# jianhao2016/AllSet

Measured on AMD Instinct MI355X. Metric: edges*d aggregated / sec (V->E->V layer fwd+bwd), higher is better.
Workload: dtype f32

## Files before the change

allset_amd/_lib.py:

```python
from __future__ import annotations

import ctypes
import os
from ctypes import c_char_p, c_float, c_int, c_int64, c_size_t, c_uint64, c_void_p, POINTER

import torch

LIB_PATH = os.path.join(os.path.dirname(os.path.abspath(__file__)), "liballset_hip.so")
ABI_VERSION = 15
CORE_ABI_VERSION = 1

SUM, MEAN, MAX, MIN = 0, 1, 2, 3
F32, BF16 = 0, 1
REDUCE_AS_TREE = 0x100
PACK_PITCH_DW, PACK_CAP = 64, 60
ARITH_AUTO, ARITH_BF16X6, ARITH_FP16X3 = 0, 1, 2
ACT_NONE, ACT_RELU, ACT_ELU = 0, 1, 2
REDUCE_CODES = {"add": SUM, "sum": SUM, "mean": MEAN, "max": MAX, "min": MIN}

_P = c_void_p
SIGNATURES = {
    "allset_version": [],
    "allset_core_version": [],
    "allset_csr_build_workspace_bytes": [c_int64, c_int64, POINTER(c_size_t)],
# ... 250 lines not shown
    "allset_spgemm_bool_fill": [_P, _P, _P, _P, c_int64, c_int64, c_int64, _P, c_int64, _P, _P, c_size_t, _P],
    "allset_loo_supported": [c_int64],
    "allset_loo_long_threshold": [],
    "allset_loo_rows": [_P, _P, _P, c_int64, _P, _P, _P, c_int64, _P, c_int64, c_int64, c_int64, c_int64, c_int64, _P],
    "allset_loo_softmax_supported": [c_int64, c_int64],
    "allset_loo_softmax_fwd": [_P, _P, _P, _P, c_int64, c_float, _P, c_int64, _P, _P, c_int64, c_int64, c_int64, c_int64, c_int64,
                               c_int64, _P],
    "allset_loo_softmax_bwd": [_P, _P, _P, _P, c_int64, c_float, _P, c_int64, _P, _P, c_int64, _P, _P, c_int64, _P, _P, _P, c_int64,
                               c_int64, c_int64, c_int64, c_int64, c_int64, _P],
    "allset_scan_rows_supported": [c_int64],
    "allset_scan_rows": [_P, _P, _P, c_int64, _P, _P, c_int64, _P, c_int64, c_int, c_int64, c_int64, c_int64, c_int64, _P],
    "allset_scan_collect": [_P, _P, _P, c_int64, _P, _P, c_int64, _P, _P, c_int, c_float, c_uint64, _P, _P, c_int64, c_int64, c_int64,
                            c_int64, c_int64, _P],
    "allset_pack_rows_f32": [_P, c_int64, _P, c_int64, c_int64, _P],
    "allset_segreduce_packed_fwd": [c_int, _P, _P, _P, _P, _P, c_int64, _P, c_int64, c_int64, c_int64, c_int64, _P],
}
EXPORTED_SYMBOLS = sorted(list(SIGNATURES) + ["allset_last_error"])


class AllSetHipError(RuntimeError):
    pass


_lib = None


def load() -> ctypes.CDLL:
    global _lib
    if _lib is not None:
        return _lib
# ... 71 lines not shown
```

allset_amd/csrc/fused_fwd2.hip:

```cpp
#include <stdlib.h>

#include "common.h"
#include "mfma.h"

namespace allset {

constexpr int kF2Block = 768;
constexpr int kF2Rows = 32;
constexpr int kF2VWaves = 8;
constexpr int kF2Sets = 4;

#ifdef ALLSET_ABL5_NOBAR
#define ALLSET_TICK() ALLSET_TICK_NO_BARRIER()
#else
#define ALLSET_TICK() ALLSET_TICK_BARRIER()
#endif

template <bool HAS_LN, bool DROP_IN, bool DROP_OUT, bool D8, bool F16, int XM = 0, bool AUX = false>
__global__ __launch_bounds__(kF2Block) void fused_linear_fwd_roles_kernel(
    const float* __restrict__ x, int64_t ldx, const float* __restrict__ gamma, const float* __restrict__ beta, float eps,
    int relu_in, float p_in, uint64_t seed_in, const float* __restrict__ W, const float* __restrict__ bias, int relu_out,
    float p_out, uint64_t seed_out, float* __restrict__ y, int64_t ldy, float* __restrict__ stats, int64_t n,
    const uint64_t* __restrict__ seed_base, uint32_t* __restrict__ mask_out, int64_t xcb, int64_t ycb, float ln_inv,
    const float* __restrict__ colb = nullptr, float* __restrict__ uo = nullptr, int64_t lduo = 0,
    const float* __restrict__ res = nullptr, int64_t ldres = 0, int relu_post = 0,
    const float* __restrict__ aux_w = nullptr, const float* __restrict__ aux_b = nullptr, float* __restrict__ aux_out = nullptr) {
  static_assert(!AUX || (XM == 0 && !DROP_IN && !HAS_LN), "auxiliary columns: the plain prologue only (behind a LayerNorm the fp16x3 form folds 2^Su into gamma / beta)");
  static_assert(XM == 0 || F16, "the tail modes are built on the fp16x3 arithmetic only");
  static_assert(XM != 1 || (HAS_LN && !DROP_IN && !DROP_OUT), "mode 1: LayerNorm prologue, no dropout");
  static_assert(XM != 2 || (!HAS_LN && !DROP_IN), "mode 2: plain operand, LayerNorm in the epilogue");
  constexpr bool ROWSC = F16 && !HAS_LN;
  constexpr bool AFF = HAS_LN || XM == 2;
  constexpr int KD = 128, ND = 128;
  constexpr int R = kF2Rows;
  constexpr int PLANE = R * 256;
  constexpr int IMG = 3 * PLANE;
  constexpr int SPY = 132;
  __shared__ __attribute__((aligned(16))) uint8_t sX[2 * IMG];
  __shared__ __attribute__((aligned(16))) float sY[2 * R * SPY];
  __shared__ __attribute__((aligned(16))) float sG[KD];
  __shared__ __attribute__((aligned(16))) float sB[KD];
  __shared__ __attribute__((aligned(16))) float sBias[ND];
  seed_in = resolve_seed(seed_base, seed_in);
// ... 240 lines not shown
          if (relu_post) { o.x = fmaxf(o.x, 0.f); o.y = fmaxf(o.y, 0.f); o.z = fmaxf(o.z, 0.f); o.w = fmaxf(o.w, 0.f); }
          if constexpr (DROP_OUT) {
            const float4 kp = keep4(seed_out, stage, hb, thr_out, keep_out);
            o.x *= kp.x; o.y *= kp.y; o.z *= kp.z; o.w *= kp.w;
          }
          if (live) *reinterpret_cast<float4*>(yb + hb * dhy + yo) = o;
        }
      }
#pragma unroll
      for (int hb = 0; hb < 2; ++hb) {
        float4 v = vv[hb];
        if constexpr (DROP_OUT && XM != 2) {
          const float4 kp = keep4(seed_out, stage, hb, thr_out, keep_out);
          v.x *= kp.x; v.y *= kp.y; v.z *= kp.z; v.w *= kp.w;
        }
#ifdef ALLSET_ABL5_NOSTORE
        if (live && v.x == 123.456f)
#else
        if (live && XM != 2)
#endif
          *reinterpret_cast<float4*>(yb + hb * dhy + yo) = v;
        if (mask_out != nullptr) {
          const uint64_t b0 = __ballot(v.x > 0.f), b1 = __ballot(v.y > 0.f), b2 = __ballot(v.z > 0.f), b3 = __ballot(v.w > 0.f);
          const int sh = 8 * (lane0 & 7);
          const uint32_t word = static_cast<uint32_t>((b0 >> sh) & 0xffu) | (static_cast<uint32_t>((b1 >> sh) & 0xffu) << 8) |
                                (static_cast<uint32_t>((b2 >> sh) & 0xffu) << 16) | (static_cast<uint32_t>((b3 >> sh) & 0xffu) << 24);
          if (lane0 < 8 && 16 * (wave >> 2) < nrows)
            mask_out[((stage * (R / 16) + (wave >> 2)) * (ND / 64) + hb) * 32 + (wave & 3) * 8 + lane0] = word;
        }
      }
      if constexpr (XM == 2) {
        __builtin_amdgcn_sched_barrier(0);
        request_res(k + 1);
        __builtin_amdgcn_sched_barrier(0);
      }
    };

    static_assert(kF2Sets == 4, "the trip below is written for four register sets");
#pragma unroll
    for (int q = 0; q < kF2Sets; ++q) request_x(q, xrS[q]);
    request_res(0);
    S0(0, xrS[0]);
    ALLSET_TICK();
// ... 199 lines not shown
    case 3: ALLSET_F2_K(false, true, true); break;
    case 4: ALLSET_F2_K(true, false, false); break;
    case 5: ALLSET_F2_K(true, false, true); break;
    case 6: ALLSET_F2_K(true, true, false); break;
    default: ALLSET_F2_K(true, true, true); break;
  }
#undef ALLSET_F2_K
#undef ALLSET_F2_KD
#undef ALLSET_F2_KE
  return 0;
}

static inline unsigned f2_grid(int64_t n) {
  const int64_t blocks = (n + kF2Rows - 1) / kF2Rows;
  return static_cast<unsigned>(blocks > 256 ? 256 : (blocks < 1 ? 1 : blocks));
}

extern "C" int allset_fused_linear_tail_supported(int64_t K, int64_t N) {
#ifdef ALLSET_NO_F16X3
  (void)K; (void)N;
  return 0;
#else
  return (K == 128 && N == 128) ? 1 : 0;
#endif
}

extern "C" int allset_fused_linear_fwd_ln_side(const float* x, int64_t ldx, const float* colb, const float* gamma, const float* beta,
                                               float eps, const float* W, const float* bias, int relu_out, float* y, int64_t ldy,
                                               float* uo, int64_t lduo, float* stats, int64_t n, int64_t K, int64_t N, void* stream) {
  clear_error();
// ... 57 lines not shown
```

allset_amd/dense.py:

```python
from __future__ import annotations

import contextlib
import os
from ctypes import byref, c_int64
from typing import Optional, Tuple

import torch
from torch.autograd.function import once_differentiable

from . import _lib
from ._lib import check, ptr, require_device, stream_of, on_device
from .ops import _ld, _rowmajor, _timed

Tensor = torch.Tensor


class _SeedSource:
    base: Optional[Tensor] = None
    salt: int = 0


_SEED_SCRATCH = torch.empty((), dtype=torch.int64)


# ... 1027 lines not shown
                                               mask is not None)):
            need = ctx.needs_input_grad
            defer = ctx.params if (_Deferred.active and (gamma is None or (need[1] and need[2])) and (not has_bias or need[4])) else None
            gx, dg, db, gw, gb = fused_linear_bwd_all(gy, mask, p_out, weight, x, stats, gamma, beta, relu_in, p_in, seed_in,
                                                      base, want_bias=need_b, defer_to=defer)
            return gx, dg, db, gw, gb, None, None, None, None, None, None, None
        if ctx.needs_input_grad[3] or need_b:
            gw, gb = wgrad_fused(gy, y, p_out, x, stats, gamma, beta, relu_in, p_in, seed_in, want_bias=need_b,
                                 seed_base=base, mask=mask)
        if ctx.needs_input_grad[0] or (gamma is not None and (ctx.needs_input_grad[1] or ctx.needs_input_grad[2])):
            gx, dg, db = fused_linear_bwd(gy, y, p_out, weight, x, stats, gamma, relu_in, p_in, seed_in, base, mask,
                                          want_gx=ctx.needs_input_grad[0])
        return gx, dg, db, gw, gb, None, None, None, None, None, None, None


class _WideNormLinear(torch.autograd.Function):

    @staticmethod
    def forward(ctx, x, gamma, beta, weight, bias, eps, relu_in, p_in, relu_out, p_out, stats_in=None, emit=None):
        seed_in = _draw_seed() if p_in > 0.0 else 0
        seed_out = _draw_seed() if p_out > 0.0 else 0
        base = _seed_base() if (p_in > 0.0 or p_out > 0.0) else None
        stats = (stats_in if stats_in is not None else row_stats(x, relu_in, eps)) if gamma is not None else None
        stats_y = torch.empty((x.shape[0], 2), dtype=torch.float32, device=x.device) if emit is not None else None
        keep_y = relu_out or p_out > 0.0
        words = activation_mask_words(x.shape[0], weight.shape[0]) if (keep_y and x.shape[0] > 0) else 0
        mask = torch.empty(words, dtype=torch.int32, device=x.device) if words > 0 else None
        y = gemm_x6(x, gemm_x6_planes(weight, False, f16=wide_f16(gamma is not None)), weight.shape[0], bias, relu_in=relu_in, stats=stats, gamma=gamma,
                    beta=beta, p_in=p_in, seed_in=seed_in, relu_out=relu_out, p_out=p_out, seed_out=seed_out, seed_base=base,
                    mask_out=mask, stats_out=stats_y, stats_eps=emit[0] if emit is not None else 1e-5,
# ... 1320 lines not shown
```

allset_amd/dist.py:

```python
from __future__ import annotations

import os
from typing import Callable, Optional, Tuple

import torch
import torch.distributed as dist
import torch.nn.functional as F

Tensor = torch.Tensor



def vertex_block(n_v: int, world: int, rank: int) -> Tuple[int, int, int]:
    per = (n_v + world - 1) // world
    return rank * per, (rank + 1) * per, per * world


def partition_hyperedges(sizes: Tensor, world: int, method: str = "contiguous") -> Tensor:
    sizes = sizes.to(torch.int64)
    n_e = sizes.numel()
    if method == "contiguous":
        csum = torch.cumsum(sizes, 0)
        total = int(csum[-1]) if n_e else 0
        mid = csum - sizes // 2
# ... 434 lines not shown
        T = inc.by_src
        return ops.pma_bwd_src(T.rowptr, T.col, alpha, V, gout, stats, slope,
                               variant=_variant(T, "pma_bwd_src", V.shape[0], V, alpha.shape[1]), row_order=T.row_order,
                               sizes=_sizes(T, V, alpha.shape[1]))


def _bn_scope(valid_rows: int, group):
    from . import dense
    return dense.sync_bn_rows(valid_rows, group)


def _valid_rows(lo: int, hi: int, n: int) -> int:
    return max(0, min(int(hi), int(n)) - int(lo))


def sharded_deepsets_layer(v2e_conv, e2v_conv, x_owned: Tensor, hg: ShardedHypergraph, aggr: str = "add",
                           dropout: float = 0.0, training: bool = False, group=None,
                           aggregate: Callable = _hip_deepsets, norm: Optional[Tensor] = None,
                           dropout_out: Optional[float] = None) -> Tensor:
    if aggr not in ("add", "sum", "mean", "max", "min"):
        raise ValueError(f"aggr {aggr!r}")
    vv = _valid_rows(hg.v_lo, hg.v_hi, hg.n_v)
    norm = hg.norm if norm is None else norm
    p_out = dropout if dropout_out is None else dropout_out
    use_halo = hg.halo is not None and hg.halo_v2e is not None
    agg_v2e, agg_e2v = _forward_aggregate(aggregate, v2e_conv), _forward_aggregate(aggregate, e2v_conv)
    with _bn_scope(vv, group):
        h = v2e_conv._mlp_act(v2e_conv.f_enc, x_owned, v2e_conv.dropout)
    if use_halo:
        e = agg_v2e(halo_gather(h, hg.halo), hg.halo_v2e, norm, aggr)
    else:
        h_full = all_gather_rows(h, group)
        e = agg_v2e(h_full, hg.v2e, norm, aggr)
    with _bn_scope(e.shape[0], group):
        e = v2e_conv._mlp_act(v2e_conv.f_dec, e, dropout)
        g = e2v_conv._mlp_act(e2v_conv.f_enc, e, e2v_conv.dropout)
    if aggr in ("max", "min") and use_halo:
        v = _HaloExtremeMerge.apply(agg_e2v(g, hg.halo_e2v, norm, aggr), hg, aggr == "min")
    elif aggr in ("max", "min"):
        partial = agg_e2v(g, hg.e2v, norm, aggr)
        v = _ShardedExtremeMerge.apply(partial, hg.local_vertex_has_incidence(), hg, group, aggr == "min")
    elif use_halo:
        v = halo_scatter_add(agg_e2v(g, hg.halo_e2v, norm, "add"), hg.halo)
    else:
        partial = agg_e2v(g, hg.e2v, norm, "add")
        v = reduce_scatter_rows(partial, group)
    if aggr == "mean":
        v = v / hg.owned_vertex_degree(group).clamp(min=1).view(-1, 1)
    with _bn_scope(vv, group):
        return e2v_conv._mlp_act(e2v_conv.f_dec, v, p_out)

# ... 752 lines not shown
```

allset_amd/functional.py:

```python
from __future__ import annotations

from typing import Optional, Tuple

import torch
from torch.autograd.function import once_differentiable

from . import _lib, ops
from ._lib import MAX, MEAN, MIN, REDUCE_CODES, SUM
from .incidence import Incidence, LeaveOneOutIncidence

Tensor = torch.Tensor


def _variant(csr, kind: str, n_rows: int, x: Tensor, heads: int = 1) -> int:
    es = x.element_size()
    wide = 16 // es
    d = x.shape[1]
    ok = (d % wide == 0 and d <= 64 * wide and x.stride(0) % wide == 0 and x.data_ptr() % 16 == 0
          and (d // max(heads, 1)) % wide == 0)
    if not ok:
        return 1
    if d * es <= 128 and csr.max_deg <= 512:
        return 2
    return csr.variant(kind, n_rows)
# ... 54 lines not shown
    return hit


_PACKED_GATHER = True


def set_packed_gather(on: bool) -> None:
    global _PACKED_GATHER
    _PACKED_GATHER = bool(on)


def packed_gather() -> bool:
    return _PACKED_GATHER


def _takes_packed(x: Tensor, w_dst: Optional[Tensor], inc: Incidence, reduce: int) -> bool:
    if not (_PACKED_GATHER and x.dtype == torch.float32 and x.dim() == 2 and x.shape[1] == 128 and x.is_contiguous()
            and x.data_ptr() % 16 == 0 and reduce in (SUM, MEAN) and w_dst is None and x.shape[0] > 0 and inc.n_dst > 0):
        return False
    csr = inc.by_dst
    return _variant(csr, "segreduce", inc.n_dst, x) == 1 and not (0 < _split(csr, x) < inc.n_dst)


class _SegReduce(torch.autograd.Function):
    @staticmethod
    def forward(ctx, x: Tensor, w_dst: Optional[Tensor], w_src: Optional[Tensor], inc: Incidence, reduce: int, packed_rows: bool = False):
        csr = inc.by_dst
        ext = reduce in (MAX, MIN)
        if packed_rows and _takes_packed(x, w_dst, inc, reduce):
            out = ops.segreduce_packed(reduce, csr.rowptr, csr.col, ops.pack_rows(x), x, inc.n_dst, row_order=csr.row_order)
            arg = None
        else:
            out, arg = ops.segreduce(reduce, csr.rowptr, csr.col, w_dst, x, inc.n_dst, want_arg=ext,
                                     variant=1 if ext else _variant(csr, "segreduce", inc.n_dst, x), row_order=csr.row_order,
                                     split=_split(csr, x))
        need_gw = w_dst is not None and ctx.needs_input_grad[1]
        ctx.inc, ctx.reduce, ctx.n_s, ctx.need_gw = inc, reduce, x.shape[0], need_gw
        ctx.save_for_backward(x if need_gw else None, w_dst, w_src, arg)
        return out

    @staticmethod
    @once_differentiable
    def backward(ctx, gout: Tensor):
        x, w_dst, w_src, arg = ctx.saved_tensors
# ... 8 lines not shown
        if ctx.needs_input_grad[0]:
            if w_dst is not None and w_src is None:
                w_src = w_dst[inc.pos_dst_of_src().long()]
            if reduce in (SUM, MEAN):
                if reduce == MEAN:
                    inv = inc.inv_count_by_src()
                    w_src = inv if w_src is None else w_src * inv
                gx, _ = ops.segreduce(SUM, T.rowptr, T.col, w_src, gout, ctx.n_s,
                                      variant=_variant(T, "segreduce", ctx.n_s, gout), row_order=T.row_order,
                                      split=_split(T, gout) if ctx.n_s == T.n_rows else -1)
            else:
                gx = ops.segmax_bwd(T.rowptr, T.col, inc.pos_dst_of_src(), w_src, arg, gout, ctx.n_s)
        if ctx.need_gw:
            csr = inc.by_dst
            gw = ops.sddmm_rowdot(reduce, csr.rowptr, csr.col, x, gout, arg)
        return gx, gw, None, None, None, None


def deepsets_aggregate(x: Tensor, inc: Incidence, norm: Optional[Tensor] = None, aggr: str = "add",
                       packed_rows: bool = False) -> Tensor:
    if aggr not in REDUCE_CODES:
        raise ValueError(f"unknown aggr {aggr!r}")
    _lib.require_device(x)
    _check_rows(x, inc)
    if norm is not None and norm.requires_grad:
        w_dst = _routed(norm, inc, True)
        w_src = _routed(norm, inc, False).detach()
    else:
        w_dst, w_src = inc.weights(norm)
    return _SegReduce.apply(x, w_dst, w_src, inc, REDUCE_CODES[aggr], bool(packed_rows))


def _loo_expand(x: Tensor, loo: LeaveOneOutIncidence, s_src: Optional[Tensor], s_seg: Optional[Tensor]) -> Tensor:
    return ops.loo_rows(loo.e_rowptr, loo.e_col, x, s_src, s_seg, long_seg=loo.long_seg if loo.n_long else None, n_long=loo.n_long)


def _loo_collect(y: Tensor, loo: LeaveOneOutIncidence, s_seg: Optional[Tensor], w_inc: Optional[Tensor], n_rows: int) -> Tensor:
    t = ops.loo_rows(loo.e_rowptr, None, y, None, s_seg, long_seg=loo.long_seg if loo.n_long else None, n_long=loo.n_long)
    out, _ = ops.segreduce(SUM, loo.v_rowptr, loo.v_col, w_inc, t, n_rows)
    return out


class _LooV2E(torch.autograd.Function):
    @staticmethod
    def forward(ctx, x: Tensor, loo: LeaveOneOutIncidence, f):
# ... 930 lines not shown
```

allset_amd/incidence.py:

```python
from __future__ import annotations

import weakref
from typing import Dict, NamedTuple, Optional, Tuple

import torch

from . import _lib, ops
from .ops import CSR

Tensor = torch.Tensor


class Incidence:

    def __init__(self, by_dst: CSR, by_src: CSR, n_src: int, n_dst: int, src_extent: int, dst_extent: int):
        self.by_dst, self.by_src = by_dst, by_src
        self.n_src, self.n_dst = int(n_src), int(n_dst)
        self.src_extent, self.dst_extent = int(src_extent), int(dst_extent)
        self.nnz = by_dst.nnz
        self.device = by_dst.rowptr.device
        self._pos_dst_of_src: Optional[Tensor] = None
        self._inv_cnt: Dict[str, Tensor] = {}
        self._wcache: Dict[Tuple, Tuple[weakref.ref, Tuple[Optional[Tensor], Optional[Tensor]]]] = {}
        self._reversed: Optional["Incidence"] = None
# ... 87 lines not shown
        if hit is not None and not entry[2] and not _capturing(norm):
            if bool((norm.reshape(-1) == 1).all()):
                hit = (None, None)
            self._wcache[key] = (entry[0], hit, True)
        if hit is None:
            flat = norm.reshape(-1)
            probed = not norm.dtype.is_floating_point
            if probed and bool((flat == 1).all()):
                hit = (None, None)
            else:
                f = flat.to(torch.float32)
                hit = (f.index_select(0, self.perm_dst_long()), f.index_select(0, self.perm_src_long()))
            self._wcache.clear()
            self._wcache[key] = (weakref.ref(norm), hit, probed)
        return hit


class LeaveOneOutIncidence:

    def __init__(self, edge_index: Tensor, n_v: Optional[int] = None, e_base: int = 0, long_threshold: Optional[int] = None):
        if edge_index.dim() != 2 or edge_index.shape[0] != 2 or edge_index.dtype != torch.int64:
            raise ValueError(f"edge_index must be int64 [2, nnz], got {edge_index.dtype} {tuple(edge_index.shape)}")
        dev = edge_index.device
        v, e = edge_index[0].contiguous(), edge_index[1].contiguous() - int(e_base)
        nnz = int(v.numel())
        if nnz >= 2 ** 31 - 1:
            raise ValueError(f"{nnz} incidences do not fit the int32 CSR")
        if nnz > 0:
            lo_v, hi_v, lo_e, hi_e = int(v.min()), int(v.max()), int(e.min()), int(e.max())
        else:
# ... 109 lines not shown
```

allset_amd/layers.py:

```python
from __future__ import annotations

import math
from typing import Tuple, Optional, Union

import os

import torch
import torch.nn as nn
import torch.nn.functional as F

from . import dense
from . import functional as AF
from .incidence import Incidence, LooDirection, cached_incidence

Tensor = torch.Tensor
EdgeIndex = Union[Tensor, Incidence]


def glorot(tensor: Optional[Tensor]) -> None:
    if tensor is not None:
        bound = math.sqrt(6.0 / (tensor.size(-2) + tensor.size(-1)))
        with torch.no_grad():
            tensor.uniform_(-bound, bound)

# ... 156 lines not shown
        return lin.weight * a.unsqueeze(0), lin.bias + lin.weight @ shift

    def _resident(self) -> bool:
        return all(dense.fused_linear_supported(lin.in_features, lin.out_features) for lin in self.lins)

    def blockable(self, x: Tensor, cb: int) -> bool:
        if cb < 4 or (cb & (cb - 1)) or not (_on_hip(x) and x.dtype == torch.float32):
            return False
        first, last = self.lins[0], self.lins[-1]
        return (all(isinstance(nm, (nn.LayerNorm, nn.Identity)) for nm in self.normalizations) and
                all(lin.bias is not None for lin in self.lins) and
                all(dense.blocked_linear_supported(lin.in_features, lin.out_features) for lin in (first, last)) and
                all(dense.fused_linear_supported(lin.in_features, lin.out_features) for lin in self.lins) and
                cb <= first.in_features // 2 and cb <= last.out_features // 2)

    def forward(self, x, _post: Optional[float] = None, _in_cb: int = 0, _out_cb: int = 0, _pre: float = 0.0):
        p = float(self.dropout) if self.training else 0.0
        post_p = (float(_post) if self.training else 0.0) if _post is not None else None
        if _pre and not self._wide_input(x):
            raise ValueError("MLP.forward(_pre=...) needs takes_pre_dropout(x)")
        if not (_in_cb or _out_cb) and self._wide_input(x):
            n0, lin0 = self.normalizations[0], self.lins[0]
            x = dense.input_norm_linear(x, n0.weight, n0.bias, lin0.weight, lin0.bias, n0.eps, float(_pre) if self.training else 0.0)
            last = len(self.lins) - 1
            if last == 0:
                return x if post_p is None else relu_dropout(x, _post, self.training)
            for i in range(1, last + 1):
                nm, lin = self.normalizations[i], self.lins[i]
                ln = nm if isinstance(nm, nn.LayerNorm) else None
                ro = i == last and post_p is not None
                x = dense.fused_norm_linear(
                    x, ln.weight if ln is not None else None, ln.bias if ln is not None else None, lin.weight, lin.bias,
                    ln.eps if ln is not None else 1e-5, relu_in=True, p_in=p, relu_out=ro, p_out=post_p if ro else 0.0)
            return x
        if _in_cb or _out_cb:
# ... 18 lines not shown
                                            relu_out=is_last and post_p is not None, p_out=0.0)
            return x
        if self._fusable(x):
            last = len(self.lins) - 1
            stats = None
            for i, lin in enumerate(self.lins):
                nm = self.normalizations[i]
                ln = nm if isinstance(nm, nn.LayerNorm) else None
                is_last = i == last
                nxt = self.normalizations[i + 1] if not is_last else None
                emit = None
                if (isinstance(nxt, nn.LayerNorm) and not (_in_cb or _out_cb)
                        and dense.wide_stats_chain_supported(lin.weight.shape[1], lin.weight.shape[0], ln is not None, i > 0, p if i > 0 else 0.0)
                        and dense.wide_linear_supported(self.lins[i + 1].weight.shape[1], self.lins[i + 1].weight.shape[0], True, True, p)):
                    emit = (nxt.eps, True)
                x = dense.fused_norm_linear(
                    x, ln.weight if ln is not None else None, ln.bias if ln is not None else None, lin.weight, lin.bias,
                    ln.eps if ln is not None else 1e-5, relu_in=i > 0, p_in=p if i > 0 else 0.0,
                    relu_out=is_last and post_p is not None, p_out=post_p if (is_last and post_p is not None) else 0.0,
                    stats_in=stats if ln is not None else None, emit_stats=emit)
                stats = None
                if emit is not None:
                    x, stats = x
            return x
        if self._bn_trainable(x):
            last = len(self.lins) - 1
            for i, lin in enumerate(self.lins):
                nm = self.normalizations[i]
                ro = i == last and post_p is not None
                po = post_p if ro else 0.0
# ... 248 lines not shown
            if norm is not None and norm.requires_grad:
                raise NotImplementedError("exclude-self data without the expansion takes no per-incidence weight (LearnMask is a parameter "
                                          "per EXPANDED incidence); expand the edge list with preprocessing.expand_edge_index instead")
            if aggr is None:
                raise ValueError("aggr was not passed!")
            x = self._mlp_act(self.f_enc, x, self.dropout, pre=_pre_dropout)
            x = AF.deepsets_aggregate_exclude_self(x, edge_index.loo, edge_index.direction, aggr, edge_index.normtype)
            return self._mlp_act(self.f_dec, x, _post_dropout if post else 0.0)
        if self.attention:
            if post and self.training:
                return self.prop(x, edge_index, _post=float(_post_dropout), _pre=float(_pre_dropout))
            x = self.prop(x, edge_index, _pre=float(_pre_dropout))
            return relu_dropout(x, _post_dropout, self.training) if post else x
        if aggr is None:
            raise ValueError("aggr was not passed!")
        x = self._mlp_act(self.f_enc, x, self.dropout, pre=_pre_dropout)
        inc = _as_incidence(edge_index, x.shape[0])
        x = AF.deepsets_aggregate(x, inc, norm, aggr, packed_rows=self.mostly_zero_enc())
        return self._mlp_act(self.f_dec, x, _post_dropout if post else 0.0)

    def _mlp_act(self, mlp, x, p, in_cb: int = 0, out_cb: int = 0, pre: float = 0.0):
        if isinstance(mlp, MLP):
            return mlp(x, _post=p, _in_cb=in_cb, _out_cb=out_cb, _pre=pre)
        return relu_dropout(mlp(x), p, self.training)
```

allset_amd/ops.py:

```python
from __future__ import annotations

from collections import defaultdict
from ctypes import byref, c_int64 as c_int64_t, c_size_t, c_void_p
from typing import Dict, List, NamedTuple, Optional, Sequence, Tuple

import torch

from . import _lib
from ._lib import check, ptr, require_device, stream_of, on_device

Tensor = torch.Tensor


class KernelTimer:

    def __init__(self):
        self.events: Dict[str, List[Tuple[torch.cuda.Event, torch.cuda.Event, int]]] = defaultdict(list)

    def summary(self) -> Dict[str, Dict[str, float]]:
        out = {}
        for name, evs in self.events.items():
            ms = [s.elapsed_time(e) for s, e, _ in evs]
            out[name] = dict(calls=len(ms), total_ms=sum(ms), avg_ms=sum(ms) / len(ms),
                             algo_bytes=sum(b for _, _, b in evs) / len(evs))
# ... 214 lines not shown
            check(lib.allset_segreduce_fwd_ex(reduce, code, variant, nnz, ptr(row_order), ptr(rowptr), ptr(col), ptr(w), ptr(x), _ld(x),
                                              ptr(out), max(d, 1), ptr(arg), n_t, n_s, d, stream_of(dev)),
                  "allset_segreduce_fwd_ex")
    return out, arg


def pack_rows(x: Tensor) -> Tensor:
    dev = require_device(x)
    _f32(x, "pack_rows")
    x = _rowmajor(x)
    n, d = x.shape
    packed = torch.empty((n, _lib.PACK_PITCH_DW), dtype=torch.int32, device=dev)
    with on_device(dev), _timed("pack_rows", dev, n * (4 * d + 4 * _lib.PACK_PITCH_DW)):
        check(_lib.load().allset_pack_rows_f32(ptr(x), _ld(x), ptr(packed), n, d, stream_of(dev)), "allset_pack_rows_f32")
    return packed


def segreduce_packed(reduce: int, rowptr: Tensor, col: Tensor, packed: Tensor, x: Tensor, n_t: int,
                     row_order: Optional[Tensor] = None) -> Tensor:
    dev = require_device(rowptr, col, packed, x)
    _f32(x, "segreduce_packed")
    x = _rowmajor(x)
    n_s, d = x.shape
    if packed.dtype != torch.int32 or tuple(packed.shape) != (n_s, _lib.PACK_PITCH_DW) or not packed.is_contiguous():
        raise _lib.AllSetHipError(f"segreduce_packed: packed must be contiguous int32[{n_s}, {_lib.PACK_PITCH_DW}] (ops.pack_rows)")
    out = torch.empty((n_t, d), dtype=x.dtype, device=dev)
    nnz = col.numel()
    algo = nnz * (4 * _lib.PACK_PITCH_DW + 4) + (n_t + 1) * 4 + n_t * d * 4
    with on_device(dev), _timed("segreduce_fwd", dev, algo):
        if row_order is not None and row_order.numel() != n_t:
# ... 1347 lines not shown
```

include/allset_hip_ext.h:

```cpp
#ifndef ALLSET_HIP_EXT_H
#define ALLSET_HIP_EXT_H

#include "allset_hip.h"

#ifdef __cplusplus
extern "C" {
#endif

#define ALLSET_ABI_VERSION 15


int allset_ln_fwd(const float* x, int64_t ldx, const float* gamma, const float* beta, float eps, int relu_in,
                  float p, uint64_t seed, float* y, int64_t ldy, float* stats, int64_t n, int64_t d,
                  const uint64_t* seed_base, void* stream);

int allset_ln_bwd_partials(int64_t n, int64_t d, int64_t* n_partials);
int allset_ln_bwd(const float* gy, int64_t ldg, const float* x, int64_t ldx, const float* stats, const float* gamma,
                  int relu_in, float p, uint64_t seed, float* gx, int64_t ldgx, float* partials, int64_t n_partials,
                  int64_t n, int64_t d, const uint64_t* seed_base, void* stream);

int allset_relu_dropout_fwd(const float* x, float p, uint64_t seed, float* y, int64_t numel,
                            const uint64_t* seed_base, void* stream);
int allset_relu_dropout_bwd(const float* gy, const float* y, float p, float* gx, int64_t numel, void* stream);

// ... 476 lines not shown
                           int64_t n_seg, int64_t n_src, int64_t nnz, int64_t d, int64_t heads, void* stream);

int allset_scan_rows_supported(int64_t d);
int allset_scan_rows(const int32_t* rowptr, const int32_t* col, const float* src, int64_t lds, const float* s_src, float* out,
                     int64_t ldo, const int32_t* long_seg, int64_t n_long, int reverse, int64_t n_seg, int64_t n_src, int64_t nnz,
                     int64_t d, void* stream);
int allset_scan_collect(const int32_t* rowptr, const int32_t* col, const float* t, int64_t ldt, const float* r_self, const float* x,
                        int64_t ldx, const float* s, const float* bias, int act, float p, uint64_t seed, const uint64_t* seed_base,
                        float* y, int64_t ldy, int64_t n_t, int64_t n_pos, int64_t d, int64_t width, void* stream);

enum { kPackPitchDw = 64, kPackCap = 60 };
int allset_pack_rows_f32(const float* x, int64_t ldx, void* packed, int64_t n, int64_t d, void* stream);
int allset_segreduce_packed_fwd(int reduce, const int32_t* row_order, const int32_t* rowptr, const int32_t* col, const void* packed,
                                const float* x, int64_t ldx, float* out, int64_t ldo, int64_t n_t, int64_t n_s, int64_t d, void* stream);

#ifdef __cplusplus
}
#endif
#endif
```

Before: 242.5 billion.

## Emit packed sparse rows directly from the fused LayerNorm-Linear epilogue

Adds a kernel mode that writes the last encoder Linear's dropout-and-ReLU output straight into the packed nonzero-row format used by the packed segment-reduce gather. The dense output is written only for rows that overflow the pack capacity, which removes the separate pack_rows pass and the full dense write of the encoder output. Python plumbing (PackedRows, takes_packed_epilogue, packs_enc) routes the packed tensor into deepsets_aggregate when the row count and incidence allow it. The cost is added epilogue work (DPP mask reduction and LDS compaction) and a narrower supported configuration.

```diff
diff --git a/allset_amd/_lib.py b/allset_amd/_lib.py
--- a/allset_amd/_lib.py
+++ b/allset_amd/_lib.py
@@ -288,6 +288,9 @@
                             c_int64, c_int64, _P],
     "allset_pack_rows_f32": [_P, c_int64, _P, c_int64, c_int64, _P],
     "allset_segreduce_packed_fwd": [c_int, _P, _P, _P, _P, _P, c_int64, _P, c_int64, c_int64, c_int64, c_int64, _P],
+    "allset_fused_linear_fwd_packed_supported": [c_int64, c_int64, c_int, c_float, c_float],
+    "allset_fused_linear_fwd_packed": [_P, c_int64, _P, _P, c_float, c_int, c_float, c_uint64, _P, _P, c_int, c_float, c_uint64, _P, _P,
+                                       c_int64, _P, c_int64, c_int64, c_int64, _P, _P, c_int, _P],
 }
 EXPORTED_SYMBOLS = sorted(list(SIGNATURES) + ["allset_last_error"])
 
diff --git a/allset_amd/csrc/fused_fwd2.hip b/allset_amd/csrc/fused_fwd2.hip
--- a/allset_amd/csrc/fused_fwd2.hip
+++ b/allset_amd/csrc/fused_fwd2.hip
@@ -26,7 +26,8 @@
     const float* __restrict__ res = nullptr, int64_t ldres = 0, int relu_post = 0,
     const float* __restrict__ aux_w = nullptr, const float* __restrict__ aux_b = nullptr, float* __restrict__ aux_out = nullptr) {
   static_assert(!AUX || (XM == 0 && !DROP_IN && !HAS_LN), "auxiliary columns: the plain prologue only (behind a LayerNorm the fp16x3 form folds 2^Su into gamma / beta)");
-  static_assert(XM == 0 || F16, "the tail modes are built on the fp16x3 arithmetic only");
+  static_assert(XM == 0 || XM == 3 || F16, "the tail modes are built on the fp16x3 arithmetic only");
+  static_assert(XM != 3 || (HAS_LN && DROP_IN && DROP_OUT && !AUX), "mode 3: LayerNorm prologue, dropout in and out");
   static_assert(XM != 1 || (HAS_LN && !DROP_IN && !DROP_OUT), "mode 1: LayerNorm prologue, no dropout");
   static_assert(XM != 2 || (!HAS_LN && !DROP_IN), "mode 2: plain operand, LayerNorm in the epilogue");
   constexpr bool ROWSC = F16 && !HAS_LN;
@@ -297,10 +298,11 @@
           const float4 kp = keep4(seed_out, stage, hb, thr_out, keep_out);
           v.x *= kp.x; v.y *= kp.y; v.z *= kp.z; v.w *= kp.w;
         }
+        if constexpr (XM == 3) vv[hb] = v;
 #ifdef ALLSET_ABL5_NOSTORE
         if (live && v.x == 123.456f)
 #else
-        if (live && XM != 2)
+        if (live && XM != 2 && XM != 3)
 #endif
           *reinterpret_cast<float4*>(yb + hb * dhy + yo) = v;
         if (mask_out != nullptr) {
@@ -310,6 +312,50 @@
                                 (static_cast<uint32_t>((b2 >> sh) & 0xffu) << 16) | (static_cast<uint32_t>((b3 >> sh) & 0xffu) << 24);
           if (lane0 < 8 && 16 * (wave >> 2) < nrows)
             mask_out[((stage * (R / 16) + (wave >> 2)) * (ND / 64) + hb) * 32 + (wave & 3) * 8 + lane0] = word;
+        }
+      }
+      if constexpr (XM == 3) {
+        uint32_t u[2][4], own[2], oth[2];
+        const uint32_t sh = 4u * (c & 7);
+#pragma unroll
+        for (int hb = 0; hb < 2; ++hb) {
+          u[hb][0] = __float_as_uint(vv[hb].x); u[hb][1] = __float_as_uint(vv[hb].y);
+          u[hb][2] = __float_as_uint(vv[hb].z); u[hb][3] = __float_as_uint(vv[hb].w);
+          const uint32_t nib = (u[hb][0] != 0u ? 1u : 0u) | (u[hb][1] != 0u ? 2u : 0u) | (u[hb][2] != 0u ? 4u : 0u) | (u[hb][3] != 0u ? 8u : 0u);
+          float mw = __uint_as_float(nib << sh);
+          mw = __uint_as_float(__float_as_uint(mw) | __float_as_uint(dpp_row<0xB1>(mw)));
+          mw = __uint_as_float(__float_as_uint(mw) | __float_as_uint(dpp_row<0x4E>(mw)));
+          mw = __uint_as_float(__float_as_uint(mw) | __float_as_uint(dpp_row<0x141>(mw)));
+          own[hb] = __float_as_uint(mw);
+          oth[hb] = __float_as_uint(dpp_row<0x140>(mw));
+        }
+        const bool hi = c >= 8;
+        const uint32_t below = (1u << sh) - 1u;
+        const int cnt0 = __popc(own[0]) + __popc(oth[0]);
+        const int kocc = cnt0 + __popc(own[1]) + __popc(oth[1]);
+        int pos[2];
+        pos[0] = 4 + (hi ? __popc(oth[0]) : 0) + __popc(own[0] & below);
+        pos[1] = 4 + cnt0 + (hi ? __popc(oth[1]) : 0) + __popc(own[1] & below);
+        uint32_t* im = reinterpret_cast<uint32_t*>(sY + (k & 1) * (R * SPY) + lr * SPY);
+        __builtin_amdgcn_fence(__ATOMIC_SEQ_CST, "wavefront");
+        __builtin_amdgcn_wave_barrier();
+        *reinterpret_cast<uint4*>(im + 4 * c) = make_uint4(0u, 0u, 0u, 0u);
+        *reinterpret_cast<uint4*>(im + (hi ? SPY - 4 : 0)) = make_uint4(own[0], oth[0], own[1], oth[1]);
+#pragma unroll
+        for (int hb = 0; hb < 2; ++hb)
+#pragma unroll
+          for (int i = 0; i < 4; ++i) {
+            const bool occ = u[hb][i] != 0u;
+            im[occ ? pos[hb] : SPY - 1] = u[hb][i];
+            pos[hb] += occ ? 1 : 0;
+          }
+        __builtin_amdgcn_fence(__ATOMIC_SEQ_CST, "wavefront");
+        __builtin_amdgcn_wave_barrier();
+        const uint4 o = *reinterpret_cast<const uint4*>(im + 4 * c);
+        if (live) *reinterpret_cast<uint4*>(reinterpret_cast<uint32_t*>(uo) + (stage * R + lr) * kPackPitchDw + 4 * c) = o;
+        if (live && kocc > kPackCap) {
+          *reinterpret_cast<float4*>(yb + yo) = vv[0];
+          *reinterpret_cast<float4*>(yb + 256 + yo) = vv[1];
         }
       }
       if constexpr (XM == 2) {
@@ -539,6 +585,52 @@
 static inline unsigned f2_grid(int64_t n) {
   const int64_t blocks = (n + kF2Rows - 1) / kF2Rows;
   return static_cast<unsigned>(blocks > 256 ? 256 : (blocks < 1 ? 1 : blocks));
+}
+
+extern "C" int allset_fused_linear_fwd_packed_supported(int64_t K, int64_t N, int has_ln, float p_in, float p_out) {
+  return (K == 128 && N == 128 && has_ln && p_in > 0.f && p_in < 1.f && p_out > 0.f && p_out < 1.f) ? 1 : 0;
+}
+
+extern "C" int allset_fused_linear_fwd_packed(const float* x, int64_t ldx, const float* gamma, const float* beta, float eps, int relu_in,
+                                              float p_in, uint64_t seed_in, const float* W, const float* bias, int relu_out, float p_out,
+                                              uint64_t seed_out, void* packed, float* side, int64_t ldside, float* stats, int64_t n,
+                                              int64_t K, int64_t N, const uint64_t* seed_base, uint32_t* mask_out, int arith,
+                                              void* stream) {
+  clear_error();
+  ALLSET_REQUIRE(n >= 0, "fused_linear_fwd_packed: negative size");
+  ALLSET_REQUIRE(arith == ALLSET_ARITH_AUTO || arith == ALLSET_ARITH_BF16X6 || arith == ALLSET_ARITH_FP16X3,
+                 "fused_linear_fwd_packed: arith must be ALLSET_ARITH_AUTO, ALLSET_ARITH_BF16X6 or ALLSET_ARITH_FP16X3");
+  if (!allset_fused_linear_fwd_packed_supported(K, N, gamma != nullptr, p_in, p_out)) {
+    set_error("fused_linear_fwd_packed: built for K = N = 128 behind a LayerNorm with dropout in and out only "
+              "(allset_fused_linear_fwd_packed_supported)");
+    return ALLSET_ERR_UNSUPPORTED;
+  }
+#ifdef ALLSET_NO_F16X3
+  if (arith == ALLSET_ARITH_FP16X3) { set_error("fused_linear_fwd_packed: this build has no fp16x3 arithmetic"); return ALLSET_ERR_UNSUPPORTED; }
+#endif
+  if (n == 0) return ALLSET_OK;
+  ALLSET_REQUIRE(x && beta && W && packed && side && stats, "fused_linear_fwd_packed: null pointer");
+  ALLSET_REQUIRE(aligned16(x) && aligned16(side) && aligned16(W) && (reinterpret_cast<uintptr_t>(stats) & 7u) == 0,
+                 "fused_linear_fwd_packed: x / side / W must be 16-byte aligned, stats 8-byte aligned");
+  ALLSET_REQUIRE((reinterpret_cast<uintptr_t>(packed) & 255u) == 0, "fused_linear_fwd_packed: the packed buffer must be 256-byte aligned");
+  ALLSET_REQUIRE(ldx >= K && ldx % 4 == 0 && ldside >= N && ldside % 4 == 0 && ldx < (1 << 24) && ldside < (1 << 24),
+                 "fused_linear_fwd_packed: rows must be 16-byte aligned, leading dimensions below 2^24");
+  const hipStream_t st = static_cast<hipStream_t>(stream);
+  const bool d8 = drop_is8(p_in) && drop_is8(p_out);
+#ifdef ALLSET_NO_F16X3
+  const bool f16 = false;
+#else
+  const bool f16 = arith != ALLSET_ARITH_BF16X6;
+#endif
+#define ALLSET_F2_PK(E8, H16)                                                                                                            \
+  fused_linear_fwd_roles_kernel<true, true, true, E8, H16, 3><<<f2_grid(n), kF2Block, 0, st>>>(                                             \
+      x, ldx, gamma, beta, eps, relu_in, p_in, seed_in, W, bias, relu_out, p_out, seed_out, side, ldside, stats, n, seed_base, mask_out, 0, 0, \
+      1.f / 128.f, nullptr, static_cast<float*>(packed), 0)
+  if (d8) { if (f16) ALLSET_F2_PK(true, true); else ALLSET_F2_PK(true, false); }
+  else    { if (f16) ALLSET_F2_PK(false, true); else ALLSET_F2_PK(false, false); }
+#undef ALLSET_F2_PK
+  ALLSET_LAUNCH_CHECK();
+  return ALLSET_OK;
 }
 
 extern "C" int allset_fused_linear_tail_supported(int64_t K, int64_t N) {
diff --git a/allset_amd/dense.py b/allset_amd/dense.py
--- a/allset_amd/dense.py
+++ b/allset_amd/dense.py
@@ -1065,6 +1065,60 @@
         return gx, dg, db, gw, gb, None, None, None, None, None, None, None
 
 
+class PackedRows:
+
+    __slots__ = ("packed", "_side")
+
+    def __init__(self, packed: Tensor, side: Tensor):
+        self.packed, self._side = packed, side
+
+    @property
+    def shape(self):
+        return self._side.shape
+
+
+class _FusedNormLinearPacked(torch.autograd.Function):
+
+    @staticmethod
+    def forward(ctx, x, gamma, beta, weight, bias, eps, relu_in, p_in, relu_out, p_out):
+        from . import ops
+        seed_in = _draw_seed()
+        seed_out = _draw_seed()
+        base = _seed_base()
+        words = activation_mask_words(x.shape[0], weight.shape[0]) if any(ctx.needs_input_grad) else 0
+        mask = torch.empty(words, dtype=torch.int32, device=x.device) if words > 0 else None
+        packed, side, stats = ops.fused_linear_fwd_packed(x, weight, bias, gamma, beta, eps, relu_in, p_in, seed_in, relu_out, p_out,
+                                                          seed_out, base, mask, _arith_for(0, weight.shape[1], weight.shape[0], True, 0))
+        ctx.save_for_backward(x, stats, gamma, beta, weight, None, mask)
+        ctx.cfg = (bool(relu_in), float(p_in), seed_in, float(p_out), bias is not None, base)
+        ctx.layout = (0, 0)
+        ctx.params = (gamma, beta, weight, bias)
+        ctx.mark_non_differentiable(packed)
+        return side, packed
+
+    @staticmethod
+    @once_differentiable
+    def backward(ctx, gy, _g_packed=None):
+        return _FusedNormLinear.backward(ctx, gy)[:10]
+
+
+def fused_norm_linear_packed_supported(x: Tensor, gamma: Optional[Tensor], weight: Tensor, p_in: float, relu_out: bool, p_out: float) -> bool:
+    from . import ops
+    N, K = weight.shape
+    return (x.is_cuda and x.dtype == torch.float32 and x.dim() == 2 and x.shape[0] > 0 and gamma is not None and bool(relu_out)
+            and ops.fused_linear_fwd_packed_supported(K, N, True, p_in, p_out))
+
+
+def fused_norm_linear_packed(x: Tensor, gamma: Tensor, beta: Tensor, weight: Tensor, bias: Optional[Tensor], eps: float, relu_in: bool,
+                             p_in: float, relu_out: bool, p_out: float) -> PackedRows:
+    if not fused_norm_linear_packed_supported(x, gamma, weight, p_in, relu_out, p_out):
+        raise _lib.AllSetHipError("fused_norm_linear_packed: built for a [128, 128] Linear behind a LayerNorm with relu_out and both "
+                                  "dropouts active only (fused_norm_linear_packed_supported)")
+    side, packed = _FusedNormLinearPacked.apply(x, gamma, beta, weight, bias, float(eps), bool(relu_in), float(p_in), bool(relu_out),
+                                                float(p_out))
+    return PackedRows(packed, side)
+
+
 class _WideNormLinear(torch.autograd.Function):
 
     @staticmethod
diff --git a/allset_amd/dist.py b/allset_amd/dist.py
--- a/allset_amd/dist.py
+++ b/allset_amd/dist.py
@@ -472,6 +472,10 @@
     return max(0, min(int(hi), int(n)) - int(lo))
 
 
+def _packs_enc(aggregate: Callable, conv, x: Tensor, inc, norm, aggr: str, group, use_halo: bool) -> bool:
+    return bool(aggregate is _hip_deepsets and not use_halo and _skip_collective(group) and conv.packs_enc(x, inc, norm, aggr))
+
+
 def sharded_deepsets_layer(v2e_conv, e2v_conv, x_owned: Tensor, hg: ShardedHypergraph, aggr: str = "add",
                            dropout: float = 0.0, training: bool = False, group=None,
                            aggregate: Callable = _hip_deepsets, norm: Optional[Tensor] = None,
@@ -483,16 +487,20 @@
     p_out = dropout if dropout_out is None else dropout_out
     use_halo = hg.halo is not None and hg.halo_v2e is not None
     agg_v2e, agg_e2v = _forward_aggregate(aggregate, v2e_conv), _forward_aggregate(aggregate, e2v_conv)
+    pk_v2e = _packs_enc(aggregate, v2e_conv, x_owned, hg.v2e, norm, aggr, group, use_halo)
     with _bn_scope(vv, group):
-        h = v2e_conv._mlp_act(v2e_conv.f_enc, x_owned, v2e_conv.dropout)
-    if use_halo:
+        h = v2e_conv._mlp_act(v2e_conv.f_enc, x_owned, v2e_conv.dropout, packed=pk_v2e)
+    if pk_v2e:
+        e = agg_v2e(h, hg.v2e, norm, aggr)
+    elif use_halo:
         e = agg_v2e(halo_gather(h, hg.halo), hg.halo_v2e, norm, aggr)
     else:
         h_full = all_gather_rows(h, group)
         e = agg_v2e(h_full, hg.v2e, norm, aggr)
     with _bn_scope(e.shape[0], group):
         e = v2e_conv._mlp_act(v2e_conv.f_dec, e, dropout)
-        g = e2v_conv._mlp_act(e2v_conv.f_enc, e, e2v_conv.dropout)
+        pk_e2v = aggr not in ("max", "min") and _packs_enc(aggregate, e2v_conv, e, hg.e2v, norm, "add", group, use_halo)
+        g = e2v_conv._mlp_act(e2v_conv.f_enc, e, e2v_conv.dropout, packed=pk_e2v)
     if aggr in ("max", "min") and use_halo:
         v = _HaloExtremeMerge.apply(agg_e2v(g, hg.halo_e2v, norm, aggr), hg, aggr == "min")
     elif aggr in ("max", "min"):
diff --git a/allset_amd/functional.py b/allset_amd/functional.py
--- a/allset_amd/functional.py
+++ b/allset_amd/functional.py
@@ -6,6 +6,7 @@
 from torch.autograd.function import once_differentiable
 
 from . import _lib, ops
+from .dense import PackedRows
 from ._lib import MAX, MEAN, MIN, REDUCE_CODES, SUM
 from .incidence import Incidence, LeaveOneOutIncidence
 
@@ -92,6 +93,51 @@
     return _PACKED_GATHER
 
 
+_PACKED_EPILOGUE = "auto"
+PACKED_EPILOGUE_MIN_ROWS = 16384
+
+
+def set_packed_epilogue(mode: str) -> None:
+    global _PACKED_EPILOGUE
+    if mode not in ("auto", "on", "off"):
+        raise ValueError(f"set_packed_epilogue: mode must be 'auto', 'on' or 'off', got {mode!r}")
+    _PACKED_EPILOGUE = mode
+
+
+def packed_epilogue() -> str:
+    return _PACKED_EPILOGUE
+
+
+class _RowsToCome:
+    dtype = torch.float32
+
+    def __init__(self, n: int):
+        self.shape = (int(n), 128)
+
+    def dim(self):
+        return 2
+
+    def is_contiguous(self):
+        return True
+
+    def data_ptr(self):
+        return 0
+
+    def element_size(self):
+        return 4
+
+    def stride(self, i):
+        return (128, 1)[i]
+
+
+def takes_packed_epilogue(n_rows: int, inc: Incidence, norm: Optional[Tensor], aggr: str) -> bool:
+    if _PACKED_EPILOGUE == "off" or (_PACKED_EPILOGUE == "auto" and n_rows < PACKED_EPILOGUE_MIN_ROWS) or aggr not in REDUCE_CODES:
+        return False
+    if not inc.known_unweighted(norm) or not (inc.src_extent <= n_rows <= inc.n_src):
+        return False
+    return _takes_packed(_RowsToCome(n_rows), None, inc, REDUCE_CODES[aggr])
+
+
 def _takes_packed(x: Tensor, w_dst: Optional[Tensor], inc: Incidence, reduce: int) -> bool:
     if not (_PACKED_GATHER and x.dtype == torch.float32 and x.dim() == 2 and x.shape[1] == 128 and x.is_contiguous()
             and x.data_ptr() % 16 == 0 and reduce in (SUM, MEAN) and w_dst is None and x.shape[0] > 0 and inc.n_dst > 0):
@@ -102,10 +148,17 @@
 
 class _SegReduce(torch.autograd.Function):
     @staticmethod
-    def forward(ctx, x: Tensor, w_dst: Optional[Tensor], w_src: Optional[Tensor], inc: Incidence, reduce: int, packed_rows: bool = False):
+    def forward(ctx, x: Tensor, w_dst: Optional[Tensor], w_src: Optional[Tensor], inc: Incidence, reduce: int, packed_rows: bool = False,
+                packed: Optional[Tensor] = None):
         csr = inc.by_dst
         ext = reduce in (MAX, MIN)
-        if packed_rows and _takes_packed(x, w_dst, inc, reduce):
+        if packed is not None:
+            if not _takes_packed(x, w_dst, inc, reduce):
+                raise _lib.AllSetHipError("deepsets_aggregate: packed rows came without a packed gather to read them "
+                                          "(functional.takes_packed_epilogue decides the route before the Linear runs)")
+            out = ops.segreduce_packed(reduce, csr.rowptr, csr.col, packed, x, inc.n_dst, row_order=csr.row_order)
+            arg = None
+        elif packed_rows and _takes_packed(x, w_dst, inc, reduce):
             out = ops.segreduce_packed(reduce, csr.rowptr, csr.col, ops.pack_rows(x), x, inc.n_dst, row_order=csr.row_order)
             arg = None
         else:
@@ -144,13 +197,16 @@
         if ctx.need_gw:
             csr = inc.by_dst
             gw = ops.sddmm_rowdot(reduce, csr.rowptr, csr.col, x, gout, arg)
-        return gx, gw, None, None, None, None
+        return gx, gw, None, None, None, None, None
 
 
 def deepsets_aggregate(x: Tensor, inc: Incidence, norm: Optional[Tensor] = None, aggr: str = "add",
                        packed_rows: bool = False) -> Tensor:
     if aggr not in REDUCE_CODES:
         raise ValueError(f"unknown aggr {aggr!r}")
+    packed = None
+    if isinstance(x, PackedRows):
+        x, packed = x._side, x.packed
     _lib.require_device(x)
     _check_rows(x, inc)
     if norm is not None and norm.requires_grad:
@@ -158,7 +214,7 @@
         w_src = _routed(norm, inc, False).detach()
     else:
         w_dst, w_src = inc.weights(norm)
-    return _SegReduce.apply(x, w_dst, w_src, inc, REDUCE_CODES[aggr], bool(packed_rows))
+    return _SegReduce.apply(x, w_dst, w_src, inc, REDUCE_CODES[aggr], bool(packed_rows), packed)
 
 
 def _loo_expand(x: Tensor, loo: LeaveOneOutIncidence, s_src: Optional[Tensor], s_seg: Optional[Tensor]) -> Tensor:
diff --git a/allset_amd/incidence.py b/allset_amd/incidence.py
--- a/allset_amd/incidence.py
+++ b/allset_amd/incidence.py
@@ -125,6 +125,16 @@
             self._wcache.clear()
             self._wcache[key] = (weakref.ref(norm), hit, probed)
         return hit
+
+    def known_unweighted(self, norm: Optional[Tensor]) -> bool:
+        if norm is None:
+            return True
+        if norm.requires_grad or norm.numel() != self.nnz:
+            return False
+        if not norm.dtype.is_floating_point:
+            return self.weights(norm)[0] is None
+        entry = self._wcache.get((norm.data_ptr(), norm._version, norm.dtype, norm.numel()))
+        return entry is not None and entry[0]() is norm and entry[1][0] is None and entry[1][1] is None
 
 
 class LeaveOneOutIncidence:
diff --git a/allset_amd/layers.py b/allset_amd/layers.py
--- a/allset_amd/layers.py
+++ b/allset_amd/layers.py
@@ -194,11 +194,25 @@
                 all(dense.fused_linear_supported(lin.in_features, lin.out_features) for lin in self.lins) and
                 cb <= first.in_features // 2 and cb <= last.out_features // 2)
 
-    def forward(self, x, _post: Optional[float] = None, _in_cb: int = 0, _out_cb: int = 0, _pre: float = 0.0):
+    def packs_output(self, x: Tensor, post: Optional[float]) -> bool:
+        if post is None or not self.training or len(self.lins) < 2 or self._forward_hooks or self._forward_pre_hooks:
+            return False
+        if nn.modules.module._global_forward_hooks or nn.modules.module._global_forward_pre_hooks:
+            return False
+        if not _on_hip(x) or x.dtype != torch.float32 or self._wide_input(x) or not self._fusable(x):
+            return False
+        nm, lin = self.normalizations[-1], self.lins[-1]
+        if not isinstance(nm, nn.LayerNorm) or nm.weight is None or nm.bias is None:
+            return False
+        return dense.fused_norm_linear_packed_supported(x, nm.weight, lin.weight, float(self.dropout), True, float(post))
+
+    def forward(self, x, _post: Optional[float] = None, _in_cb: int = 0, _out_cb: int = 0, _pre: float = 0.0, _packed_out: bool = False):
         p = float(self.dropout) if self.training else 0.0
         post_p = (float(_post) if self.training else 0.0) if _post is not None else None
         if _pre and not self._wide_input(x):
             raise ValueError("MLP.forward(_pre=...) needs takes_pre_dropout(x)")
+        if _packed_out and (_in_cb or _out_cb or _pre or not self.packs_output(x, _post)):
+            raise ValueError("MLP.forward(_packed_out=True) needs packs_output(x, _post)")
         if not (_in_cb or _out_cb) and self._wide_input(x):
             n0, lin0 = self.normalizations[0], self.lins[0]
             x = dense.input_norm_linear(x, n0.weight, n0.bias, lin0.weight, lin0.bias, n0.eps, float(_pre) if self.training else 0.0)
@@ -247,6 +261,9 @@
                         and dense.wide_stats_chain_supported(lin.weight.shape[1], lin.weight.shape[0], ln is not None, i > 0, p if i > 0 else 0.0)
                         and dense.wide_linear_supported(self.lins[i + 1].weight.shape[1], self.lins[i + 1].weight.shape[0], True, True, p)):
                     emit = (nxt.eps, True)
+                if is_last and _packed_out:
+                    return dense.fused_norm_linear_packed(x, ln.weight, ln.bias, lin.weight, lin.bias, ln.eps, relu_in=True, p_in=p,
+                                                          relu_out=True, p_out=post_p)
                 x = dense.fused_norm_linear(
                     x, ln.weight if ln is not None else None, ln.bias if ln is not None else None, lin.weight, lin.bias,
                     ln.eps if ln is not None else 1e-5, relu_in=i > 0, p_in=p if i > 0 else 0.0,
@@ -525,12 +542,18 @@
             return relu_dropout(x, _post_dropout, self.training) if post else x
         if aggr is None:
             raise ValueError("aggr was not passed!")
-        x = self._mlp_act(self.f_enc, x, self.dropout, pre=_pre_dropout)
         inc = _as_incidence(edge_index, x.shape[0])
+        x = self._mlp_act(self.f_enc, x, self.dropout, pre=_pre_dropout, packed=self.packs_enc(x, inc, norm, aggr, _pre_dropout))
         x = AF.deepsets_aggregate(x, inc, norm, aggr, packed_rows=self.mostly_zero_enc())
         return self._mlp_act(self.f_dec, x, _post_dropout if post else 0.0)
 
-    def _mlp_act(self, mlp, x, p, in_cb: int = 0, out_cb: int = 0, pre: float = 0.0):
+    def packs_enc(self, x: Tensor, inc, norm, aggr, pre: float = 0.0) -> bool:
+        return bool(self.mostly_zero_enc() and not pre and isinstance(self.f_enc, MLP) and x.dim() == 2
+                    and AF.takes_packed_epilogue(x.shape[0], inc, norm, aggr) and self.f_enc.packs_output(x, self.dropout))
+
+    def _mlp_act(self, mlp, x, p, in_cb: int = 0, out_cb: int = 0, pre: float = 0.0, packed: bool = False):
         if isinstance(mlp, MLP):
+            if packed:
+                return mlp(x, _post=p, _pre=pre, _packed_out=True)
             return mlp(x, _post=p, _in_cb=in_cb, _out_cb=out_cb, _pre=pre)
         return relu_dropout(mlp(x), p, self.training)
diff --git a/allset_amd/ops.py b/allset_amd/ops.py
--- a/allset_amd/ops.py
+++ b/allset_amd/ops.py
@@ -252,6 +252,32 @@
     with on_device(dev), _timed("pack_rows", dev, n * (4 * d + 4 * _lib.PACK_PITCH_DW)):
         check(_lib.load().allset_pack_rows_f32(ptr(x), _ld(x), ptr(packed), n, d, stream_of(dev)), "allset_pack_rows_f32")
     return packed
+
+
+def fused_linear_fwd_packed_supported(K: int, N: int, has_ln: bool, p_in: float, p_out: float) -> bool:
+    return bool(_lib.load().allset_fused_linear_fwd_packed_supported(int(K), int(N), int(has_ln), float(p_in), float(p_out)))
+
+
+def fused_linear_fwd_packed(x: Tensor, weight: Tensor, bias: Optional[Tensor], gamma: Tensor, beta: Tensor, eps: float, relu_in: bool,
+                            p_in: float, seed_in: int, relu_out: bool, p_out: float, seed_out: int, seed_base: Optional[Tensor],
+                            mask_out: Optional[Tensor], arith: int = 0) -> Tuple[Tensor, Tensor, Tensor]:
+    dev = require_device(x, weight, bias, gamma, beta)
+    for t in (x, weight, bias, gamma, beta):
+        if t is not None:
+            _f32(t, "fused_linear_fwd_packed")
+    x = _rowmajor(x)
+    n, K = x.shape
+    N = weight.shape[0]
+    packed = torch.empty((n, _lib.PACK_PITCH_DW), dtype=torch.int32, device=dev)
+    side = torch.empty((n, N), dtype=torch.float32, device=dev)
+    stats = torch.empty((n, 2), dtype=torch.float32, device=dev)
+    nparam = weight.numel() + N + 2 * K
+    with on_device(dev), _timed("fused_linear_fwd", dev, n * (4 * K + 4 * _lib.PACK_PITCH_DW) + 4 * nparam):
+        check(_lib.load().allset_fused_linear_fwd_packed(
+            ptr(x), _ld(x), ptr(gamma.contiguous()), ptr(beta.contiguous()), eps, int(relu_in), p_in, seed_in, ptr(weight.contiguous()),
+            ptr(bias.contiguous() if bias is not None else None), int(relu_out), p_out, seed_out, ptr(packed), ptr(side), max(N, 1),
+            ptr(stats), n, K, N, ptr(seed_base), ptr(mask_out), int(arith), stream_of(dev)), "allset_fused_linear_fwd_packed")
+    return packed, side, stats
 
 
 def segreduce_packed(reduce: int, rowptr: Tensor, col: Tensor, packed: Tensor, x: Tensor, n_t: int,
diff --git a/include/allset_hip_ext.h b/include/allset_hip_ext.h
--- a/include/allset_hip_ext.h
+++ b/include/allset_hip_ext.h
@@ -514,6 +514,12 @@
 int allset_segreduce_packed_fwd(int reduce, const int32_t* row_order, const int32_t* rowptr, const int32_t* col, const void* packed,
                                 const float* x, int64_t ldx, float* out, int64_t ldo, int64_t n_t, int64_t n_s, int64_t d, void* stream);
 
+int allset_fused_linear_fwd_packed_supported(int64_t K, int64_t N, int has_ln, float p_in, float p_out);
+int allset_fused_linear_fwd_packed(const float* x, int64_t ldx, const float* gamma, const float* beta, float eps, int relu_in,
+                                   float p_in, uint64_t seed_in, const float* W, const float* bias, int relu_out, float p_out,
+                                   uint64_t seed_out, void* packed, float* side, int64_t ldside, float* stats, int64_t n, int64_t K,
+                                   int64_t N, const uint64_t* seed_base, uint32_t* mask_out, int arith, void* stream);
+
 #ifdef __cplusplus
 }
 #endif
```

New measurement: 246.5 billion (median of 6 runs). 1.02x the previous value.
